# xindonglin99/allsteps_isaaclab

Measured on AMD Instinct MI355X. Metric: env-steps/sec (whole node), Allsteps-v0 at 4096 envs, 1/2/4/8 MI355X, higher is better.
Workload: dtype f32; 1 GPU; Allsteps-v0 biped walker, 4096 envs/GPU, stone curriculum level 0, decimation 4 x dt 1/240; num_envs_per_gpu=4096, global_envs=4096, parallelism=dp1 (env shards, no collective in step)

## Files before the change

### allsteps_isaaclab_amd/csrc/allsteps_abi.hip

```cpp
#include <hip/hip_runtime.h>

#include <algorithm>
#include <cstdlib>
#include <cstdio>
#include <cstring>
#include <string>
#include <vector>

#include "../../include/allsteps.h"
#include "allsteps_kernels.h"

namespace {

thread_local std::string g_err;

int fail(int code, const std::string& msg) {
  g_err = msg;
  return code;
}

#define HIP_TRY(expr)                                                                        \
  do {                                                                                       \
    hipError_t _e = (expr);                                                                  \
    if (_e != hipSuccess) return fail(AS_ERR_HIP, std::string(#expr ": ") + hipGetErrorString(_e)); \
// ... 123 lines not shown
  hipDeviceProp_t prop;
  HIP_TRY(hipGetDeviceProperties(&prop, device));
  if (std::strncmp(prop.gcnArchName, "gfx950", 6) != 0)
    return fail(AS_ERR_NO_DEVICE, std::string("as_create: device is ") + prop.gcnArchName + ", built for gfx950");

  as::Consts h{};
  h.model = *model;
  h.sim = *sim;
  h.task = *task;
  h.nv = 6 + model->num_hinges;
  h.act.mode = AS_ACT_TORQUE;
  h.st_has_hind = state->contact_mask_hind != nullptr;
  const int nl = model->num_links;
  for (int i = 0; i < nl; ++i) {
    int pa = model->parent[i];
    if (i == 0 ? pa != -1 : (pa < 0 || pa >= i)) return fail(AS_ERR_INVALID, "as_create: parent not topological");
    h.lpath[i] = (i == 0 ? 0u : h.lpath[pa]) | (1u << i);
    if (i > 0 && pa == 0) h.root_kids |= 1u << i;
  }
  for (int i = 0; i < nl; ++i)
    for (int l = 0; l < nl; ++l)
      if ((h.lpath[l] >> i) & 1u) h.lsub[i] |= 1u << l;
  for (int j = 0; j < h.nv; ++j) h.dsub[j] = j < 6 ? h.lsub[0] : h.lsub[j - 5];
  for (int i = 0; i < nl; ++i) {
    h.max_path = std::max(h.max_path, __builtin_popcount(h.lpath[i]) - 1);
    if (i > 0) h.max_sub = std::max(h.max_sub, __builtin_popcount(h.lsub[i]) - 1);
  }
  while ((1 << h.fk_rounds) < h.max_path) ++h.fk_rounds;
  if (h.fk_rounds > 4) return fail(AS_ERR_INVALID, "as_create: tree deeper than 16 links");
  for (int i = 0; i < nl; ++i) {
    int a = i > 0 ? model->parent[i] : 0;
    for (int r = 0; r < 4; ++r) {
      h.jump[i] |= (uint32_t)a << (8 * r);
      for (int k = 0; k < (1 << r); ++k) a = a > 0 ? model->parent[a] : 0;
    }
  }
  for (int k = 0; k < model->num_hinges; ++k) {
    int li = model->cfg_dof_link[k];
    if (li < 1 || li >= model->num_links) return fail(AS_ERR_INVALID, "as_create: cfg_dof_link");
  }
  for (int l = 0; l < model->num_links; ++l) {
    uint32_t mask = 0x3Fu;
    for (int i = l; i > 0; i = model->parent[i]) mask |= 1u << (6 + i - 1);
    h.ancmask[l] = mask;
  }
  for (int j = 0; j < h.nv; ++j)
    for (int k = 0; k < h.nv; ++k) {
      const int lk = k < 6 ? 0 : k - 5;
      if ((h.ancmask[lk] >> j) & 1u) h.ddesc[j] |= 1u << k;
    }
  if (!as::step_supported_nv(h.nv))
    return fail(AS_ERR_INVALID, "as_create: no k_step instantiation for " + std::to_string(h.nv) + " dofs");
  as::fill_lane_table(h);

  as_env* env = new as_env();
  env->n = num_envs;
  env->device = device;
  env->seed = seed;
  env->env_offset = env_id_offset;
  env->st = *state;
  env->num_steps = task->num_steps;
  env->nv = h.nv;
  env->host = h;
  env->sweep_skip = as_sweep_plan(model, nullptr) == 1;
  if (hipMalloc(&env->consts_dev, sizeof(as::Consts)) != hipSuccess ||
      hipMalloc(&env->counters_dev, 2 * as::kCntBank * sizeof(int32_t)) != hipSuccess ||
      hipMalloc(&env->side_dev, (size_t)as::kSideWords * num_envs * sizeof(uint32_t)) != hipSuccess) {
    (void)hipFree(env->consts_dev);
    (void)hipFree(env->counters_dev);
    delete env;
    return fail(AS_ERR_HIP, "as_create: hipMalloc failed");
  }
  HIP_TRY(hipMemcpy(env->consts_dev, &h, sizeof(as::Consts), hipMemcpyHostToDevice));
  HIP_TRY(hipMemset(env->counters_dev, 0, 2 * as::kCntBank * sizeof(int32_t)));
  HIP_TRY(hipMemset(env->side_dev, 0, (size_t)as::kSideWords * num_envs * sizeof(uint32_t)));
  const char* wm = std::getenv("ALLSTEPS_WAVE_MAP");
  if (as::wave_map_fits(num_envs) && !(wm && std::strcmp(wm, "0") == 0)) {
    env->map_streamed = num_envs / 2 > 8 * prop.multiProcessorCount && !(wm && std::strcmp(wm, "resident") == 0);
    std::vector<int32_t> map((size_t)num_envs);
    for (int w = 0; w < num_envs / as::kMapEnvs; ++w)
      for (int t = 0; t < as::kMapEnvs; ++t)
        map[(size_t)2 * as::wave_map_block(w, t >> 1, num_envs, env->map_streamed) + (t & 1)] = w * as::kMapEnvs + t;
    if (hipMalloc(&env->wave_map_dev, map.size() * sizeof(int32_t)) != hipSuccess) {
      (void)as_destroy(env);
      return fail(AS_ERR_HIP, "as_create: hipMalloc failed");
    }
    HIP_TRY(hipMemcpy(env->wave_map_dev, map.data(), map.size() * sizeof(int32_t), hipMemcpyHostToDevice));
  }
  *out = env;
  return AS_OK;
}

int as_destroy(as_env_t* env) {
  if (!env) return AS_OK;
  (void)hipSetDevice(env->device);
  for (hipEvent_t e : env->ev) (void)hipEventDestroy(e);
  (void)hipFree(env->consts_dev);
  (void)hipFree(env->counters_dev);
  (void)hipFree(env->side_dev);
  (void)hipFree(env->wave_map_dev);
  delete env;
  return AS_OK;
}

static int run(as_env_t* env, int mode, const float* actions, float* obs, float* reward, uint8_t* term,
               uint8_t* trunc, const float* reset_draws, void* stream, const uint8_t* reset_mask = nullptr) {
// ... 274 lines not shown
```

### allsteps_isaaclab_amd/csrc/allsteps_kernels.h

```cpp
#pragma once

#include <hip/hip_runtime.h>
#include <stdint.h>

#include "../../include/allsteps.h"
#include "allsteps_lane_table.h"

namespace as {

constexpr int kMaxLinks = 24;
constexpr int kMaxDofs = 6 + kMaxLinks - 1;

enum { kModeStep = 0, kModeReset = 1, kModePhysics = 2, kModeTask = 3 };

struct Consts {
  as_model_t model;
  as_sim_t sim;
  as_task_t task;
  as_actuator_t act;
  as_quad_task_t quad;
  int32_t nv;
  int32_t st_has_hind;
  int32_t max_path;
  int32_t max_sub;
  uint32_t root_kids;
  uint32_t lpath[kMaxLinks];
  uint32_t lsub[kMaxLinks];
  uint32_t ancmask[kMaxLinks];
  uint32_t dsub[kMaxDofs];
  uint32_t ddesc[kMaxDofs];
  uint32_t jump[kMaxLinks];
  int32_t fk_rounds;
  LaneRow lane[kLaneRows];
};
static_assert(kLaneRows == 32 && kMaxLinks <= kLaneRows && kMaxDofs <= kLaneRows, "one table row per k_step lane");
inline void fill_lane_table(Consts& c) {
  build_lane_table(c.lane, c.model, c.task, c.act, c.nv, c.lpath, c.lsub, c.ancmask, c.dsub, c.jump);
}

struct StepArgs {
  const Consts* consts;
  as_state_t st;
  int32_t n;
  int32_t mode;
  const float* actions;
  float* reward;
  float* obs;
  uint32_t* side;
  uint8_t* terminated;
  uint8_t* truncated;
  const float* reset_draws;
  const uint8_t* reset_mask;
  int32_t* counters;
  uint64_t seed;
  int64_t env_offset;
  unsigned long long* stamps;
  const int32_t* wave_map;
};

enum {
  kStLoad = 0, kStFK, kStLinkQ, kStDyn, kStChol, kStSolve, kStCollide, kStRows, kStWsolve, kStPGS,
  kStIntegrate, kStFKFinal, kStTask, kStReset, kStStore, kNumStamps
};

constexpr int kCntSlots = 16;
constexpr int kCntStride = 16;
constexpr int kCntBank = kCntStride * (1 + kCntSlots);

constexpr int kSideState = 9;
constexpr int kSideObs = 11;
constexpr int kSideRegen = kSideState + kSideObs;
constexpr int kSideCost = kSideRegen + 1;
constexpr int kSideWords = kSideCost + 1;

constexpr int kMapEnvs = 64;
__host__ __device__ inline bool wave_map_fits(int n) { return n > 0 && n % (8 * kMapEnvs) == 0; }
__host__ __device__ inline int wave_map_block(int w, int p, int n, bool streamed) {
  const int C = n / kMapEnvs;
  if (streamed || p < kMapEnvs / 4) return p * C + w;
  return (n >> 2) + (kMapEnvs / 2 - 1 - p) * C + w;
}
constexpr int kCntLevel = 2;
constexpr int kCntDropped = 3;

struct QuadArgs {
// ... 63 lines not shown
```

### allsteps_isaaclab_amd/csrc/allsteps_kernels.hip

```cpp
#include <hip/hip_runtime.h>

#include "../../include/allsteps.h"
#include "allsteps_device.h"
#include "allsteps_kernels.h"

namespace as {

constexpr int G = 32;
constexpr int EPB = 2;
constexpr int LMAX = kMaxLinks;
constexpr int NVMAX = 6 + LMAX - 1;
constexpr int MAXC = AS_MAX_CONTACTS;
constexpr int MAXR = AS_MAX_ROWS;
constexpr int NST = AS_NUM_STONES;
constexpr int kBisectIters = 12;
constexpr int kPairsPerChunk = G;
static_assert(kPairsPerChunk - 1 + G <= 64, "pending pair list (PhaseScratch::col.pl)");
constexpr int kSweepB = 4;
typedef float v4f __attribute__((ext_vector_type(4)));
typedef float v2f __attribute__((ext_vector_type(2)));

static_assert(NVMAX <= G, "one lane per generalized velocity");
static_assert(LMAX <= G, "one lane per link");
static_assert(MAXR <= G, "one row per lane in the row builders");
// ... 155 lines not shown

__device__ __forceinline__ int half_scan3(int c, int& total) {
  const int sh = threadIdx.x & 32;
  const uint32_t m0 = (uint32_t)(__ballot((c & 1) != 0) >> sh);
  const uint32_t m1 = (uint32_t)(__ballot((c & 2) != 0) >> sh);
  const uint32_t lt = (1u << (threadIdx.x & 31)) - 1u;
  total = __popc(m0) + 2 * __popc(m1);
  return __popc(m0 & lt) + 2 * __popc(m1 & lt);
}

template <int CTRL>
__device__ __forceinline__ uint32_t dpp_u(uint32_t v) {
  return (uint32_t)__builtin_amdgcn_update_dpp(0, (int)v, CTRL, 0xF, 0xF, true);
}

__device__ __forceinline__ void half_or2(uint32_t& x, uint32_t& y) {
  const auto s = __builtin_amdgcn_permlane16_swap((int)x, (int)y, false, false);
  uint32_t c = (uint32_t)s[0] | (uint32_t)s[1];
  c |= dpp_u<0xB1>(c);
  c |= dpp_u<0x4E>(c);
  c |= dpp_u<0x141>(c);
  c |= dpp_u<0x140>(c);
  const auto t = __builtin_amdgcn_permlane16_swap((int)c, (int)c, false, false);
  x = (uint32_t)t[0];
  y = (uint32_t)t[1];
}

template <int N>
__device__ __forceinline__ void half_min_n(float (&v)[N]) {
  static_assert(N % 2 == 0, "pairs");
  constexpr int P = N / 2;
  float c[P];
#pragma unroll
  for (int p = 0; p < P; ++p) {
    const auto s = __builtin_amdgcn_permlane16_swap(__float_as_int(v[2 * p]), __float_as_int(v[2 * p + 1]), false, false);
    c[p] = fminf(__int_as_float(s[0]), __int_as_float(s[1]));
  }
#pragma unroll
  for (int p = 0; p < P; ++p) c[p] = fminf(c[p], dpp<0xB1>(c[p]));
#pragma unroll
  for (int p = 0; p < P; ++p) c[p] = fminf(c[p], dpp<0x4E>(c[p]));
#pragma unroll
  for (int p = 0; p < P; ++p) c[p] = fminf(c[p], dpp<0x141>(c[p]));
#pragma unroll
  for (int p = 0; p < P; ++p) c[p] = fminf(c[p], dpp<0x140>(c[p]));
#pragma unroll
  for (int p = 0; p < P; ++p) {
    const auto s = __builtin_amdgcn_permlane16_swap(__float_as_int(c[p]), __float_as_int(c[p]), false, false);
    v[2 * p] = __int_as_float(s[0]);
    v[2 * p + 1] = __int_as_float(s[1]);
  }
}

constexpr int kWaveRecFlag = 31, kWaveRecBase = 64, kWaveRecWords = 26;
static_assert(16 + kNumStamps <= kWaveRecFlag && kNumStamps + 11 <= kWaveRecWords, "stamp slots");
struct Stamp {
  unsigned long long* p;
  unsigned long long* acc;
  unsigned long long t;
  unsigned long long t0 = 0ull, rt0 = 0ull;
  unsigned rows = 0u, cons = 0u;
  __device__ void start() {
    if (p) {
      if (threadIdx.x < kNumStamps) acc[threadIdx.x] = 0ull;
      t = t0 = __builtin_amdgcn_s_memtime();
      rt0 = __builtin_amdgcn_s_memrealtime();
      __syncthreads();
    }
  }
  __device__ void count(int nrow, int nc) {
    if (p) {
      rows += (unsigned)nrow;
      cons += (unsigned)nc;
    }
  }
  __device__ void mark(int k) {
    if (p) {
      unsigned long long now = __builtin_amdgcn_s_memtime();
      if (threadIdx.x == 0) acc[k] += now - t;
      t = now;
    }
  }
  __device__ void flush() {
    if (p) {
      __syncthreads();
      unsigned long long tot = 0;
      for (int k = 0; k < kNumStamps; ++k) tot += acc[k];
      if (p[kWaveRecFlag]) {
        unsigned long long* rec = p + kWaveRecBase + (size_t)blockIdx.x * kWaveRecWords;
        const unsigned long long now = __builtin_amdgcn_s_memtime();
        const unsigned hw = __builtin_amdgcn_s_getreg((31 << 11) | 4);
        const unsigned xcc = __builtin_amdgcn_s_getreg((31 << 11) | 20);
        const int k = threadIdx.x;
        if (k < kNumStamps) rec[k] = acc[k];
        if (k == 0) {
          rec[kNumStamps] = tot; rec[kNumStamps + 1] = t0; rec[kNumStamps + 2] = now;
          rec[kNumStamps + 9] = rt0; rec[kNumStamps + 10] = __builtin_amdgcn_s_memrealtime();
          rec[kNumStamps + 3] = hw; rec[kNumStamps + 4] = xcc;
          rec[kNumStamps + 5] = rows; rec[kNumStamps + 7] = cons;
        }
        if (k == 32) { rec[kNumStamps + 6] = rows; rec[kNumStamps + 8] = cons; }
      } else {
        if (threadIdx.x < kNumStamps) {
          atomicAdd(p + threadIdx.x, acc[threadIdx.x]);
          atomicMax(p + 16 + threadIdx.x, acc[threadIdx.x]);
        }
        if (threadIdx.x == 0) atomicMax(p + kNumStamps, tot);
      }
    }
  }
};

__device__ __forceinline__ int take_bit(uint32_t& m, bool& valid) {
  valid = m != 0u;
  const int l = valid ? __builtin_ctz(m) : 0;
  m &= m - 1u;
  return l;
}

constexpr int kZeroRow = LMAX - 1;
static_assert(AS_ACT_DIM + 1 <= kZeroRow, "zero row past the links");
__device__ __forceinline__ int take_bit_z(uint32_t& m) {
  const int l = m != 0u ? __builtin_ctz(m) : kZeroRow;
  m &= m - 1u;
  return l;
}

template <int W, int U>
__device__ __forceinline__ void path_sum(uint32_t mask, int n_max, float (&acc)[W], const float (*rows)[W]) {
  for (int it = 0; it < n_max; it += U) {
    int l[U];
#pragma unroll
    for (int u = 0; u < U; ++u) l[u] = take_bit_z(mask);
    float x[U][W];
#pragma unroll
    for (int u = 0; u < U; ++u)
#pragma unroll
      for (int k = 0; k < W; ++k) x[u][k] = rows[l[u]][k];
#pragma unroll
    for (int u = 0; u < U; ++u)
#pragma unroll
      for (int k = 0; k < W; ++k) acc[k] += x[u][k];
  }
}

struct LinkC {
  float oq[4], ax[3], an[3], op[3];
};
__device__ __forceinline__ LinkC load_link(const Consts& K, int lane) {
  const as_model_t& m = K.model;
  const int i = lane >= 1 && lane < m.num_links ? lane : 0;
  LinkC c;
#pragma unroll
  for (int k = 0; k < 4; ++k) c.oq[k] = m.offset_quat[i][k];
// ... 455 lines not shown
                             const float* n, float sep, float r) {
  if (slot >= ncap) return;
  s.clink[slot] = link; s.clink2[slot] = link2; s.cstone[slot] = stone; s.cfoot[slot] = foot; s.csep[slot] = sep;
  for (int k = 0; k < 3; ++k) { s.cn[slot][k] = n[k]; s.cpt[slot][k] = P[k] - n[k] * r; }
}

struct GeomC {
  int link, type, foot;
  float r, p0[3], p1[3];
  uint32_t anc;
};
__device__ __forceinline__ float capsule_contact_sel(const float* a1, const float* b1, float r1, const float* a2,
                                                     const float* b2, float r2, float* P, float* n) {
  float d1[3], d2[3], r[3];
#pragma unroll
  for (int k = 0; k < 3; ++k) {
    d1[k] = b1[k] - a1[k];
    d2[k] = b2[k] - a2[k];
    r[k] = a1[k] - a2[k];
  }
  const float a = as_dot3(d1, d1), e = as_dot3(d2, d2), f = as_dot3(d2, r);
  const float eps = 1e-12f;
  const bool pa = a <= eps, pe = e <= eps, gen = !pa && !pe;
  const float c = as_dot3(d1, r);
  const float b = as_dot3(d1, d2);
  const float den = fmaf(a, e, -(b * b));
  const float sm = den > 0.f ? as_clamp01(fmaf(b, f, -(c * e)) / den) : 0.f;
  const float tq = (pa ? f : fmaf(b, sm, f)) / e;
  const bool lo = gen && tq < 0.f, hi = gen && tq > 1.f;
  const float sq = as_clamp01((hi ? b - c : -c) / a);
  const float s = pa ? 0.f : (pe || lo || hi) ? sq : sm;
  const float t = pa ? (pe ? 0.f : as_clamp01(tq)) : pe ? 0.f : lo ? 0.f : hi ? 1.f : tq;
  float c1[3], c2[3], w[3];
#pragma unroll
  for (int k = 0; k < 3; ++k) {
    c1[k] = fmaf(s, d1[k], a1[k]);
    c2[k] = fmaf(t, d2[k], a2[k]);
    w[k] = c1[k] - c2[k];
  }
  const float dist = sqrtf(as_dot3(w, w));
  const bool nz = dist > 1e-9f;
  const float inv = 1.0f / dist;
  n[0] = nz ? w[0] * inv : 0.f;
  n[1] = nz ? w[1] * inv : 0.f;
  n[2] = nz ? w[2] * inv : 1.f;
  const float sep = dist - r1 - r2;
  const float off = fmaf(0.5f, sep, r2);
#pragma unroll
  for (int k = 0; k < 3; ++k) P[k] = fmaf(off, n[k], c2[k]);
  return sep;
}

__device__ __forceinline__ int collide(const Consts& K, EnvS& s, int lane, int ncap, const GeomC& gc, const float* h,
                                       float margin) {
  const as_model_t& m = K.model;
  const int nst = K.task.num_steps, ng = m.num_geoms, npri = m.num_priority_geoms, nsp = m.num_self_pairs;
  constexpr int kSelfW = AS_MAX_SELF_PAIRS / G;
  int spw[kSelfW];
#pragma unroll
  for (int i = 0; i < kSelfW; ++i) spw[i] = G * i + lane < nsp ? m.self_pair[G * i + lane] : 0;
  const bool gv = lane < ng;
  const int link = gc.link, gtype = gc.type, foot = gc.foot;
  const float r = gc.r;
  float a[3], bb[3];
  {
    float t0[3], t1[3];
    matvec3(s.R[link], gc.p0, t0);
    matvec3(s.R[link], gc.p1, t1);
    for (int k = 0; k < 3; ++k) { a[k] = s.p[link][k] + t0[k]; bb[k] = s.p[link][k] + t1[k]; }
  }
  const float L = sqrtf((bb[0] - a[0]) * (bb[0] - a[0]) + (bb[1] - a[1]) * (bb[1] - a[1]) +
                        (bb[2] - a[2]) * (bb[2] - a[2]));
  const float mid[3] = {0.5f * (a[0] + bb[0]), 0.5f * (a[1] + bb[1]), 0.5f * (a[2] + bb[2])};
  float blo[3], bhi[3], ext[6];
#pragma unroll
  for (int k = 0; k < 3; ++k) {
    const float e = gtype == 0 ? a[k] : fminf(a[k], bb[k]);
    const float f = gtype == 0 ? a[k] : fmaxf(a[k], bb[k]);
    ext[k] = gv ? e - r : 1e30f;
    ext[3 + k] = gv ? -(f + r) : 1e30f;
  }
  half_min_n(ext);
#pragma unroll
  for (int k = 0; k < 3; ++k) {
    blo[k] = ext[k] - margin;
    bhi[k] = -ext[3 + k] + margin;
  }
  bool isc = false;
  float cst[3] = {0.f, 0.f, 0.f};
  if (lane < nst) {
    isc = true;
#pragma unroll
    for (int k = 0; k < 3; ++k) {
      cst[k] = s.stones[3 * lane + k] - s.root_pos[k];
      isc = isc && (cst[k] - h[k] <= bhi[k]) && (cst[k] + h[k] >= blo[k]);
    }
  }
  uint64_t bal = __ballot(isc);
  const int half = (threadIdx.x >> 5) & 1;
  uint32_t mine = (uint32_t)(bal >> (32 * half));
  if (isc) {
    const int pos = __popc(mine & ((1u << lane) - 1u));
    s.cand[pos] = lane;
    *reinterpret_cast<v4f*>(s.x.col.cc[pos]) = v4f{cst[0], cst[1], cst[2], 0.f};
  }
  const int ncand = __popc(mine);
  {
// ... 26 lines not shown
    for (int k = 0; k < 3; ++k) c[k] = s.stones[3 * pst + k] - s.root_pos[k];
    float lo = 0.f, hi = 1.f;
#pragma unroll 4
    for (int it = 0; it < kBisectIters; ++it) {
      const float t = 0.5f * (lo + hi);
      const bool up = sd_box_slope(A, Bb, t, c, h) > 0.f;
      hi = up ? t : hi;
      lo = up ? lo : t;
    }
    if (act) {
      float n0[3];
      const float s0 = sd_box(A, c, h, n0) - pr;
      if (pty == 0) {
        if (s0 < margin) {
          for (int k = 0; k < 3; ++k) { P0[k] = A[k]; N0[k] = n0[k]; }
          SEP0 = s0;
          cnt = 1;
        }
      } else {
        float n1[3];
        float s1 = sd_box(Bb, c, h, n1) - pr;
        float ts = 0.5f * (lo + hi), Ps[3], ns[3];
        for (int k = 0; k < 3; ++k) Ps[k] = A[k] + ts * (Bb[k] - A[k]);
        float ss = sd_box(Ps, c, h, ns) - pr;
        bool e0 = s0 < margin, e1 = s1 < margin;
        bool es = ss < margin && ss < fminf(s0, s1) - 0.002f;
        for (int k = 0; k < 3; ++k) { P0[k] = A[k]; N0[k] = n0[k]; }
        SEP0 = s0;
        if (e0) {
          for (int k = 0; k < 3; ++k) { P1[k] = Bb[k]; N1[k] = n1[k]; P2[k] = Ps[k]; N2[k] = ns[k]; }
          SEP1 = s1; SEP2 = ss;
          if (!e1) { for (int k = 0; k < 3; ++k) { P1[k] = Ps[k]; N1[k] = ns[k]; } SEP1 = ss; }
        } else {
          for (int k = 0; k < 3; ++k) { P0[k] = Bb[k]; N0[k] = n1[k]; P1[k] = Ps[k]; N1[k] = ns[k]; }
          SEP0 = s1; SEP1 = ss;
          if (!e1) { for (int k = 0; k < 3; ++k) { P0[k] = Ps[k]; N0[k] = ns[k]; } SEP0 = ss; }
        }
        cnt = (int)e0 + (int)e1 + (int)es;
      }
    }
    int total;
    const int slot = base + half_scan3(cnt, total);
    if (cnt > 0) emit_contact(s, slot, ncap, plink, -1, pst, pfoot, P0, N0, SEP0, pr);
    if (cnt > 1) emit_contact(s, slot + 1, ncap, plink, -1, pst, pfoot, P1, N1, SEP1, pr);
    if (cnt > 2) emit_contact(s, slot + 2, ncap, plink, -1, pst, pfoot, P2, N2, SEP2, pr);
    base += total;
    const int rest = pend - npairs;
    const int tail = lane < rest ? pl[npairs + lane] : 0;
    __syncthreads();
    if (lane < rest) pl[lane] = tail;
    pend = rest;
    __syncthreads();
  };
  __syncthreads();
  uint32_t* cneed = s.x.col.need;
  const float pa[3] = {gtype == 0 ? a[0] : mid[0], gtype == 0 ? a[1] : mid[1], gtype == 0 ? a[2] : mid[2]};
  const float cap_lim = 0.5f * L + r + margin;
#pragma unroll 1
  for (int ci = 0; ci < ncand; ++ci) {
    const v4f cv = *reinterpret_cast<const v4f*>(s.x.col.cc[ci]);
    const float c[3] = {cv.x, cv.y, cv.z};
    float nr[3];
    const float sd = sd_box(pa, c, h, nr);
    bool need = false;
    if (gv) need = gtype == 0 ? sd - r < margin : sd <= cap_lim;
    const uint32_t bl = (uint32_t)(__ballot(need) >> (32 * half));
    if (lane == 0) cneed[ci] = bl;
  }
  __syncthreads();
  const uint32_t primask = npri >= 32 ? ~0u : (1u << npri) - 1u;
  const int wcand = max(__builtin_amdgcn_readlane(ncand, 0), __builtin_amdgcn_readlane(ncand, 32));
#pragma unroll 1
  for (int cls = 0; cls < 2; ++cls) {
#pragma unroll 1
    for (int ci = 0; ci < wcand; ++ci) {
      const uint32_t bl = ci < ncand ? cneed[ci] & (cls == 0 ? primask : ~primask) : 0u;
      if ((bl >> lane) & 1u) pl[pend + __popc(bl & ((1u << lane) - 1u))] = (s.cand[ci] << 8) | lane;
      pend += __popc(bl);
      if (max(__builtin_amdgcn_readlane(pend, 0), __builtin_amdgcn_readlane(pend, 32)) >= kPairsPerChunk)
        flush(pend < kPairsPerChunk ? pend : kPairsPerChunk);
    }
  }
  if (pend > 0) flush(pend);
  pend = 0;
  auto flush_self = [&](int npairs) {
    const bool act = lane < npairs;
    const int e = pl[act ? lane : 0];
    const int g1 = e & 0xff, g2 = e >> 8;
    int cnt = 0, l1 = 0, l2 = 0;
    float P[3], n[3], sep = 0.f;
    if (act) {
      const float* q1 = s.x.col.g[g1];
      const float* q2 = s.x.col.g[g2];
      sep = capsule_contact_sel(q1, q1 + 3, q1[6], q2, q2 + 3, q2[6], P, n);
      cnt = sep < margin;
      l1 = __float_as_int(q1[7]) >> 8;
      l2 = __float_as_int(q2[7]) >> 8;
    }
    int total;
    const int slot = base + half_scan3(cnt, total);
    if (cnt) emit_contact(s, slot, ncap, l1, l2, -1, -1, P, n, sep, 0.f);
    base += total;
    const int rest = pend - npairs;
    const int tail = lane < rest ? pl[npairs + lane] : 0;
    __syncthreads();
    if (lane < rest) pl[lane] = tail;
    pend = rest;
    __syncthreads();
  };
  uint32_t hbl[kSelfW];
  static_assert(kSelfW % 4 == 0, "batches of four words");
#pragma unroll
  for (int i = 0; i < kSelfW; ++i) hbl[i] = 0u;
#pragma unroll
  for (int i0 = 0; i0 < kSelfW; i0 += 4) {
    if (G * i0 >= nsp) break;
    v4f s1[4], s2[4];
#pragma unroll
    for (int i = 0; i < 4; ++i) {
      s1[i] = *reinterpret_cast<const v4f*>(s.x.col.bs[spw[i0 + i] & 0xff]);
      s2[i] = *reinterpret_cast<const v4f*>(s.x.col.bs[spw[i0 + i] >> 8]);
    }
    asm volatile("" : "+v"(s1[0]), "+v"(s1[1]), "+v"(s1[2]), "+v"(s1[3]), "+v"(s2[0]), "+v"(s2[1]), "+v"(s2[2]),
                 "+v"(s2[3]));
#pragma unroll
    for (int i = 0; i < 4; ++i) {
      const bool pv = G * (i0 + i) + lane < nsp;
      const float m1[3] = {s1[i].x, s1[i].y, s1[i].z}, m2[3] = {s2[i].x, s2[i].y, s2[i].z};
      const bool hit = as_sphere_bound(m1, s1[i].w, m2, s2[i].w, margin);
      hbl[i0 + i] = (uint32_t)(__ballot(pv & hit) >> (32 * half));
    }
  }
  const uint32_t lt = (1u << lane) - 1u;
  int tot = 0, at[kSelfW];
#pragma unroll
  for (int i = 0; i < kSelfW; ++i) {
// ... 192 lines not shown
    s.tau[lane] = as_dc_motor(s.qt[lane], s.qi[lane], s.u[6 + lane], A.stiffness, A.damping, A.saturation_effort,
                              A.effort_limit, A.velocity_limit);
  }
  fk<true>(K, s, lane, tp, lc, smp);
  ts.mark(kStFK);
  float Sj[6], Fj[6];
  dynamics<NV>(K, s, lane, tp, K.sim.gravity, Sj, Fj, smp);
  ts.mark(kStLinkQ);
  typedef SweepLayout<NV> SL;
  constexpr int NP = SL::NP;
  float Hr[NP];
  h_row<NV>(s, lane, tp, gc.anc, Sj, Fj, *reinterpret_cast<float(*)[NV]>(Hr));
  ts.mark(kStDyn);
  {
    float Hs[NP];
#pragma unroll
    for (int k = 0; k < NV; ++k) Hs[SL::pos(SL::padded(k))] = Hr[k];
#pragma unroll
    for (int q = 0; q < NP - NV; ++q) Hs[SL::pos(SL::PAD + q)] = lane == NV + q ? 1.f : 0.f;
    sweep_inverse<NV, SKIP>(s, lane, Hs);
#pragma unroll
    for (int k = 0; k < NV; ++k) Hr[k] = lane < NV ? -Hs[SL::pos(SL::padded(k))] : 0.f;
#pragma unroll
    for (int k = NV; k < NP; ++k) Hr[k] = 0.f;
  }
  ts.mark(kStChol);
  float uj = 0.f;
  {
    float acc = 0.f;
#pragma unroll
    for (int k = 0; k < NV; ++k) acc = fmaf(Hr[k], s.b[k], acc);
    if (lane < NV) {
      uj = fmaf(dt, acc, s.u[lane]);
      s.u[lane] = uj;
    }
  }
  __syncthreads();
  ts.mark(kStSolve);
  int lo_v = 0, hi_v = 0;
  float err_lo = 0.f, err_hi = 0.f;
  if (lane < nh) {
    float qv = s.qi[lane], pred = qv + dt * s.u[6 + lane];
    err_lo = tp.lo - qv;
    err_hi = qv - tp.hi;
    lo_v = pred < tp.lo;
    hi_v = pred > tp.hi;
  }
  int ltotal;
  const int lpos = half_scan3(lo_v + hi_v, ltotal);
  const int nlim = ltotal < MAXR ? ltotal : MAXR;
  const int ncap = (MAXR - nlim) / 3 < MAXC ? (MAXR - nlim) / 3 : MAXC;
  float sb = K.sim.baumgarte, ssl = K.sim.slop, smd = K.sim.max_depen_vel, sfr = K.sim.friction, smg = K.sim.margin;
  float sh[3] = {K.sim.stone_half[0], K.sim.stone_half[1], K.sim.stone_half[2]};
  asm volatile("" : "+s"(sb), "+s"(ssl), "+s"(smd), "+s"(sfr), "+s"(smg), "+s"(sh[0]), "+s"(sh[1]), "+s"(sh[2]));
  const int nc = collide(K, s, lane, ncap, gc, sh, smg);
  ts.mark(kStCollide);

  if (lane < nc) {
    float t1[3], t2[3];
    tangents(s.cn[lane], t1, t2);
    const float* dirs[3] = {s.cn[lane], t1, t2};
    float sp = s.csep[lane];
    const int lk = s.clink[lane] | ((s.clink2[lane] + 1) << 8);
    for (int d = 0; d < 3; ++d) {
      int r = 3 * lane + d;
      for (int k = 0; k < 3; ++k) s.cdir[lane][d][k] = dirs[d][k];
      s.rlink[r] = lk;
      s.rsign[r] = 0.f;
      const float num = sp < 0.f ? sb * fmaxf(-sp - ssl, 0.f) : -sp;
      const float tv = num / dt;
      s.rmeta[r][1] = d == 0 ? (sp < 0.f ? fminf(tv, smd) : tv) : 0.f;
      s.rmeta[r][2] = d == 1 ? sfr : 0.f;
    }
  }
  const int crow = 3 * nc;
  int slot = crow + lpos;
  for (int sd = 0; sd < 2; ++sd) {
    int viol = sd == 0 ? lo_v : hi_v;
    if (!viol) continue;
    if (slot < MAXR) {
      float err = sd == 0 ? err_lo : err_hi;
      s.rlink[slot] = -1 - (6 + lane);
      s.rsign[slot] = sd == 0 ? 1.f : -1.f;
      const float tv = (err > 0.f ? sb * err : err) / dt;
      s.rmeta[slot][1] = err > 0.f ? fminf(tv, smd) : tv;
      s.rmeta[slot][2] = slot % 3 == 2 ? __builtin_inff() : 0.f;
    }
    ++slot;
  }
  const int nrow = crow + nlim;
  ts.count(nrow, nc);
  if (lane == 0) s.nrows += nrow;
  const int maxrow = max(__builtin_amdgcn_readlane(nrow, 0), __builtin_amdgcn_readlane(nrow, 32));
  __syncthreads();
  {
    const int lvl = __builtin_amdgcn_readfirstlane(maxrow) / kPrioRows;
    if (lvl >= 3) __builtin_amdgcn_s_setprio(3);
    else if (lvl == 2) __builtin_amdgcn_s_setprio(2);
    else if (lvl == 1) __builtin_amdgcn_s_setprio(1);
    else __builtin_amdgcn_s_setprio(0);
  }
  v2f Jr[LDJ / 2];
  uint32_t jmask = ~0u;
  {
    const int rr = lane < MAXR ? lane : 0;
    const int c = rr / 3, u = rr - 3 * c;
    const int lk = s.rlink[rr];
    const float sg = s.rsign[rr];
// ... 95 lines not shown
    half_or2(b[2], b[3]);
#pragma unroll
    for (int k = 0; k < 4; ++k) mask_out[k] = b[k];
  }
  float rq[4], rp[3];
  {
    const float* u = s.u;
    float c0w[3];
    for (int k = 0; k < 3; ++k) c0w[k] = fmaf(dt, u[k], s.root_pos[k] + s.c0[k]);
    const float* w = u + 3;
    const float wn = sqrtf(dot3(w, w));
    const float th = wn * dt;
    float sn, cs;
    as_sincosf(0.5f * th, &sn, &cs);
    const float sc = sn / wn;
    const bool big = th > 1e-12f;
    const float dq[4] = {big ? cs : 1.f, big ? w[0] * sc : 0.5f * dt * w[0], big ? w[1] * sc : 0.5f * dt * w[1],
                         big ? w[2] * sc : 0.5f * dt * w[2]};
    const float* q0 = s.root_quat;
    float nq[4] = {dq[0] * q0[0] - dq[1] * q0[1] - dq[2] * q0[2] - dq[3] * q0[3],
                   dq[0] * q0[1] + dq[1] * q0[0] + dq[2] * q0[3] - dq[3] * q0[2],
                   dq[0] * q0[2] - dq[1] * q0[3] + dq[2] * q0[0] + dq[3] * q0[1],
                   dq[0] * q0[3] + dq[1] * q0[2] - dq[2] * q0[1] + dq[3] * q0[0]};
    const float qn = 1.0f / sqrtf(nq[0] * nq[0] + nq[1] * nq[1] + nq[2] * nq[2] + nq[3] * nq[3]);
    for (int k = 0; k < 4; ++k) rq[k] = nq[k] * qn;
    float Rn[9], cl[3];
    quat_to_mat(rq, Rn);
    matvec3(Rn, m.com[0], cl);
    for (int k = 0; k < 3; ++k) rp[k] = c0w[k] - cl[k];
  }
  if (lane < nh) {
    float v = fminf(fmaxf(s.u[6 + lane], -K.sim.max_joint_vel), K.sim.max_joint_vel);
    s.u[6 + lane] = v;
    s.qi[lane] = fmaf(dt, v, s.qi[lane]);
  }
  if (lane == 0) {
    for (int k = 0; k < 4; ++k) s.root_quat[k] = rq[k];
    for (int k = 0; k < 3; ++k) s.root_pos[k] = rp[k];
  }
  __syncthreads();
  ts.mark(kStIntegrate);
}


struct Useful {
  float h, roll, pitch, body_dist, dist_s;
  int reached;
};

template <class TaskT>
__device__ void compute_useful(TaskT& T, const float* root_pos, const float* root_quat, const float* bp,
                               const float* stones_env, int stride, uint32_t mask_r, uint32_t mask_l, int& idx,
                               int& prev, int& next, int& count, int& swing, float& pot, float& old_pot,
                               float* foot_contact, bool tick, Useful& u) {
  const int N = T.num_steps;
  float lower = fminf(bp[8], bp[5]);
  u.h = bp[2] - lower;
  euler_rp_from_quat(root_quat, &u.roll, &u.pitch);
  u.reached = 0;
  u.dist_s = 0.f;
  if (tick) {
    float cf0 = ((mask_r >> idx) & 1u) ? 1.f : 0.f;
    float cf1 = ((mask_l >> idx) & 1u) ? 1.f : 0.f;
    foot_contact[0] = cf0;
    foot_contact[1] = cf1;
    float tx = stones_env[(idx * 3 + 0) * stride], ty = stones_env[(idx * 3 + 1) * stride];
    float dx0 = bp[3] - tx, dy0 = bp[4] - ty, dx1 = bp[6] - tx, dy1 = bp[7] - ty;
    float d0 = sqrtf(dx0 * dx0 + dy0 * dy0), d1 = sqrtf(dx1 * dx1 + dy1 * dy1);
    float cfs = swing == 0 ? cf0 : cf1;
    float ds = swing == 0 ? d0 : d1;
    u.reached = (cfs > 0.f) && (ds < T.step_radius);
    if (u.reached) count += 1;
    if (count >= T.stop_frames) {
      swing ^= 1;
      int ni = min(max(idx + 1, 0), N - 1);
      idx = ni;
      prev = min(max(ni - 1, 0), N - 1);
      next = min(max(ni + 1, 0), N - 1);
      count = 0;
    }
    u.dist_s = swing == 0 ? d0 : d1;
  }
  float dx = stones_env[(next * 3 + 0) * stride] - root_pos[0];
  float dy = stones_env[(next * 3 + 1) * stride] - root_pos[1];
  u.body_dist = sqrtf(dx * dx + dy * dy);
  old_pot = pot;
  pot = -(u.body_dist) / T.step_dt;
}

__device__ __forceinline__ int xcd_block(int b, int nb) {
  const int q = nb >> 3, r = nb & 7, x = b & 7, slot = b >> 3;
  return (x < r ? x * (q + 1) : r * (q + 1) + (x - r) * q) + slot;
}

constexpr int kStepThreads = 64;
static_assert(kStepThreads == 64, "k_step assumes a one-wave (wave64) workgroup: see the FK rounds");

template <int NV, uint64_t SKIP>
__global__ __launch_bounds__(kStepThreads) __attribute__((amdgpu_waves_per_eu(2, 2))) void k_step(StepArgs P) {
  __shared__ Smem sm;
  CK* Kc = (CK*)P.consts;
  const Consts& K = *(const Consts*)Kc;
  const int el = threadIdx.x >> 5, lane = threadIdx.x & 31;
  const int n = P.n;
  EnvS& s = sm.env[el];
  const as_state_t& st = P.st;
  Stamp ts{P.stamps, sm.stamp_acc, 0ull};
  ts.start();
  int e_raw = xcd_block(blockIdx.x, gridDim.x) * EPB + el;
  if (P.wave_map) e_raw = P.wave_map[EPB * blockIdx.x + el];
  const ConstV4* rowp = (const ConstV4*)&Kc->lane[lane];
// ... 66 lines not shown
  if (lane < 4) s.root_quat[lane] = v_rq;
  if (lane == 0) { s.ndrop = 0; s.nrows = 0; }
  if (lane < nh) {
    int i = (int)rc[9].w - 1;
    s.qi[i] = v_q;
    s.u[6 + i] = v_qd;
    float a = fminf(fmaxf(v_a, -1.f), 1.f);
    s.act[lane] = a;
    s.tau[i] = gain * row_gear * a;
    s.qt[i] = Kc->act.action_scale * a + row_dq;
  }
  if (lane < ns3) s.stones[lane] = v_s0;
  if (lane + G < ns3) s.stones[lane + G] = v_s1;
  if (lane < kPkWords) s.pk[lane] = v_pk;
  __syncthreads();
  ts.mark(kStLoad);
  const bool do_physics = P.mode == kModeStep || P.mode == kModePhysics;
  if (do_physics) {
    const int substeps = Kc->sim.substeps;
    for (int sub = 0; sub < substeps; ++sub) substep<NV, SKIP>(K, sm, s, lane, tp, gc, lc, mask, ts);
  }
  const u32x4* rowg = (const u32x4*)&K.lane[lane];
  const u32x4 rr8 = rowg[8], rr9 = rowg[9];
  const float rs_q = __uint_as_float(rr8.z), rs_qm = __uint_as_float(rr8.w), rs_sg = __uint_as_float(rr9.x);
  const float rs_lo = __uint_as_float(rr9.y), rs_hi = __uint_as_float(rr9.z);
  const int rs_li = (int)rr9.w;
  float rd_m = 0.f, rd_n = 0.f;
  if (P.reset_draws && P.mode != kModePhysics) {
    rd_m = P.reset_draws[(size_t)e * 22];
    rd_n = P.reset_draws[(size_t)e * 22 + 1 + lh];
  }
  asm volatile("" ::: "memory");
  if (do_physics) {
    fk<false>(*Kc, s, lane, tp, lc, Kc->max_path);
    if (lane == 0) { s.mask[0] = mask[0]; s.mask[1] = mask[1]; s.mask[2] = mask[2]; s.mask[3] = mask[3]; }
  }
  ts.mark(kStFKFinal);
  if (lane == 0 && !do_physics) { s.mask[0] = mask[0]; s.mask[1] = mask[1]; }
  __syncthreads();
  float bp[9];
  if (do_physics) {
    const int ls[3] = {m.torso_link, m.foot_link[0], m.foot_link[1]};
    for (int b = 0; b < 3; ++b)
      for (int k = 0; k < 3; ++k) bp[3 * b + k] = s.root_pos[k] + s.p[ls[b]][k];
  } else {
    for (int k = 0; k < 9; ++k) bp[k] = __uint_as_float(s.pk[kPkBody + k]);
  }
  int idx = (int)s.pk[kPkIdx], prev = (int)s.pk[kPkPrev], next = (int)s.pk[kPkNext], count = (int)s.pk[kPkCount];
  int swing = (int)s.pk[kPkSwing], ep_len = (int)s.pk[kPkEpLen];
  float pot = __uint_as_float(s.pk[kPkPot]), old_pot = __uint_as_float(s.pk[kPkOldPot]);
  float fc[2] = {__uint_as_float(s.pk[kPkFc0]), __uint_as_float(s.pk[kPkFc1])};
  uint32_t episode = s.pk[kPkEpisode];
  bool done = false;
  if (P.mode == kModeStep || P.mode == kModeTask) {
    ep_len += 1;
    Useful u;
    compute_useful(T, s.root_pos, s.root_quat, bp, s.stones, 1, s.mask[0], s.mask[1], idx, prev, next, count,
                   swing, pot, old_pot, fc, true, u);
    float a2 = 0.f, en = 0.f;
    int atlim = 0;
    if (lane < nh) {
      const int li = rs_li;
      float a = s.act[lane];
      a2 = a * a;
      en = fabsf(s.u[6 + li - 1] * a);
      atlim = fabsf(scale_transform(s.qi[li - 1], rs_lo, rs_hi)) > 0.99f;
    }
    a2 = half_sum(a2);
    en = half_sum(en);
    uint64_t bl = __ballot(atlim != 0);
    int nlim = __popcll(bl >> (32 * el) & 0xffffffffull);
    const float* lv = s.u;
    float speed = sqrtf(lv[0] * lv[0] + lv[1] * lv[1] + lv[2] * lv[2]);
    bool time_out = ep_len >= T.max_episode_length - 1;
    bool fell = u.h < term_h;
    bool so_fast = speed > 5.0f;
    bool died = s.root_pos[2] < T.fall_abs;
    bool terminated = fell || so_fast || died;
    float progress = pot - old_pot;
    bool roll_v = (u.roll > 0.4f) || (u.roll < -0.4f);
    bool pitch_v = (u.pitch > 0.4f) || (u.pitch < -0.2f);
    float roll_cost = roll_v ? fabsf(u.roll) : 0.f;
    float pitch_cost = pitch_v ? fabsf(u.pitch) : 0.f;
    float speed_cost = speed > 1.6f ? speed - 1.6f : 0.f;
    float action_cost = T.action * sqrtf(a2);
    float energy_cost = T.energy * en;
    float limit_cost = (float)nlim * T.joint_limit;
    bool cond = u.reached && count == 1 && idx < T.num_steps - 1;
    float step_rew = cond ? 50.0f * as_expf(-u.dist_s / 0.25f) : 0.f;
    bool bonus_c = idx == T.num_steps - 1 && u.body_dist < 0.15f;
    float total = T.alive + progress;
    total = total - roll_cost;
    total = total - pitch_cost;
    total = total - speed_cost;
    total = total - energy_cost;
    total = total - action_cost;
    total = total - limit_cost;
    total = total + step_rew;
    total = total + (bonus_c ? 10.0f : 0.f);
    float rew = terminated ? T.death : total;
    done = terminated || time_out;
    if (valid && lane == 0) {
      P.reward[e] = rew;
      P.terminated[e] = terminated ? 1 : 0;
      P.truncated[e] = time_out ? 1 : 0;
    }
  } else if (P.mode == kModeReset) {
    done = P.reset_mask == nullptr || P.reset_mask[e] != 0;
  }
// ... 19 lines not shown
      float dm = rd_m, dn = rd_n;
      if (!P.reset_draws) {
        float blk[4];
        philox_block(P.seed, (uint32_t)(P.env_offset + e), episode, 0u, kResetTag, blk);
        dm = blk[0];
        if (lane < nh) {
          const int k = 1 + lane;
          philox_block(P.seed, (uint32_t)(P.env_offset + e), episode, (uint32_t)(k >> 2), kResetTag, blk);
          const int sl = k & 3;
          dn = sl == 0 ? blk[0] : (sl == 1 ? blk[1] : (sl == 2 ? blk[2] : blk[3]));
        }
      }
      ep_len = 0;
      old_pot = 0.f; pot = 0.f; count = 0; swing = 0; idx = 1; prev = 0; next = 2;
      const bool mirror = dm > 0.5f;
      if (mirror) swing ^= 1;
      if (lane < nh) {
        const float sign = mirror ? rs_sg : 1.f;
        float jp = mirror ? rs_qm : rs_q;
        float jv = 0.f * sign;
        int li = rs_li;
        float x = jp + (dn * (T.noise_hi - T.noise_lo) + T.noise_lo);
        float sc = fminf(fmaxf(scale_transform(x, rs_lo, rs_hi), T.clip_lo), T.clip_hi);
        s.qi[li - 1] = unscale_transform(sc, rs_lo, rs_hi);
        s.u[6 + li - 1] = jv;
      }
      if (lane < 3) {
        const float ir[3] = {T.init_root[0], T.init_root[1], T.init_root[2]};
        s.root_pos[lane] = lane == 0 ? ir[0] : (lane == 1 ? ir[1] : ir[2]);
        s.u[lane] = 0.f;
        s.u[3 + lane] = 0.f;
      }
      if (lane == 0) {
        float sg = mirror ? -1.f : 1.f;
        s.root_quat[0] = 1.f;
        s.root_quat[1] = 0.f * sg;
        s.root_quat[2] = 0.f * sg;
        s.root_quat[3] = 0.f * sg;
      }
      episode += 1u;
    }
    __syncthreads();
    fk<false>(*Kc, s, lane, tp, lc, Kc->max_path);
    if (done) {
      const int ls[3] = {m.torso_link, m.foot_link[0], m.foot_link[1]};
      for (int b = 0; b < 3; ++b)
        for (int k = 0; k < 3; ++k) bp[3 * b + k] = s.root_pos[k] + s.p[ls[b]][k];
    }
  }
  __syncthreads();
  if (P.obs) {
    int i2 = idx, p2 = prev, n2 = next, c2 = count, w2 = swing;
    float pot2 = pot, op2 = old_pot, fc2[2] = {fc[0], fc[1]};
    Useful u2;
    compute_useful(T, s.root_pos, s.root_quat, bp, s.stones, 1, s.mask[0], s.mask[1], i2, p2, n2, c2, w2, pot2,
                   op2, fc2, true, u2);
    float* ob = s.x.obs;
    uint32_t* side = P.side;
    if (lane == 0) {
      ob[0] = u2.h;
      ob[1] = u2.roll;
      ob[2] = u2.pitch;
      float vb[3];
      quat_rotate_inverse(s.root_quat, s.u, vb);
      ob[3] = vb[0]; ob[4] = vb[1]; ob[5] = vb[2];
      ob[48] = fc2[0];
      ob[49] = fc2[1];
    }
    if (lane < nh) {
      const int li = rs_li;
      ob[6 + lane] = scale_transform(s.qi[li - 1], rs_lo, rs_hi);
      ob[27 + lane] = fminf(fmaxf(s.u[6 + li - 1] * T.dof_vel_scale, -5.f), 5.f);
    }
    if (lane < 6) {
      const int t = lane < 3 ? lane : lane - 3;
      const int ti = lane < 3 ? (t == 0 ? p2 : (t == 1 ? i2 : n2)) : (t == 0 ? prev : (t == 1 ? idx : next));
      const float tw[3] = {s.stones[3 * ti], s.stones[3 * ti + 1], s.stones[3 * ti + 2]};
      float o3[3];
      subtract_frame_transforms(s.root_pos, s.root_quat, tw, o3);
      if (lane < 3) {
        for (int k = 0; k < 3; ++k) ob[50 + 3 * t + k] = o3[k];
      } else if (valid) {
        for (int k = 0; k < 3; ++k) side[(kSideState + 2 + 3 * t + k) * n + e] = __float_as_uint(o3[k]);
      }
    }
    __syncthreads();
    if (valid) {
      float* orow = P.obs + (size_t)e * AS_OBS_DIM;
      orow[lane] = ob[lane];
      if (lane < AS_OBS_DIM - 32) orow[32 + lane] = ob[32 + lane];
      if (lane == 0) {
        const uint32_t sv[kSideState + 2] = {(uint32_t)idx, (uint32_t)prev, (uint32_t)next, (uint32_t)count,
                                             (uint32_t)swing, __float_as_uint(pot), __float_as_uint(old_pot),
                                             __float_as_uint(fc[0]), __float_as_uint(fc[1]),
                                             __float_as_uint(fc[0]), __float_as_uint(fc[1])};
        for (int k = 0; k < kSideState + 2; ++k) side[k * n + e] = sv[k];
        side[kSideRegen * n + e] = regen ? 1u : 0u;
      }
    }
    idx = i2; prev = p2; next = n2; count = c2; swing = w2;
    pot = pot2; old_pot = op2; fc[0] = fc2[0]; fc[1] = fc2[1];
  }
  ts.mark(kStReset);
  if (valid) {
    if (lane < 3) {
      st.root_pos[lane * n + e] = s.root_pos[lane];
      st.root_lin[lane * n + e] = s.u[lane];
      st.root_ang[lane * n + e] = s.u[3 + lane];
    }
// ... 584 lines not shown
```

Before: 34.79 million env-steps/s.

## Split bisection of leftover collision pairs across lane groups

```diff
diff --git a/allsteps_isaaclab_amd/csrc/allsteps_abi.hip b/allsteps_isaaclab_amd/csrc/allsteps_abi.hip
--- a/allsteps_isaaclab_amd/csrc/allsteps_abi.hip
+++ b/allsteps_isaaclab_amd/csrc/allsteps_abi.hip
@@ -199,6 +199,12 @@
   if (!as::step_supported_nv(h.nv))
     return fail(AS_ERR_INVALID, "as_create: no k_step instantiation for " + std::to_string(h.nv) + " dofs");
   as::fill_lane_table(h);
+  h.pair_group_cap = 4;
+  if (const char* pg = std::getenv("ALLSTEPS_PAIR_GROUP")) {
+    if (std::strlen(pg) != 1 || pg[0] < '1' || pg[0] > '4')
+      return fail(AS_ERR_INVALID, std::string("as_create: ALLSTEPS_PAIR_GROUP=") + pg + ", expected 1, 2, 3 or 4");
+    h.pair_group_cap = pg[0] - '0';
+  }
 
   as_env* env = new as_env();
   env->n = num_envs;
diff --git a/allsteps_isaaclab_amd/csrc/allsteps_kernels.h b/allsteps_isaaclab_amd/csrc/allsteps_kernels.h
--- a/allsteps_isaaclab_amd/csrc/allsteps_kernels.h
+++ b/allsteps_isaaclab_amd/csrc/allsteps_kernels.h
@@ -5,6 +5,7 @@
 
 #include "../../include/allsteps.h"
 #include "allsteps_lane_table.h"
+#include "allsteps_pair_group.h"
 
 namespace as {
 
@@ -31,6 +32,7 @@
   uint32_t ddesc[kMaxDofs];
   uint32_t jump[kMaxLinks];
   int32_t fk_rounds;
+  int32_t pair_group_cap;
   LaneRow lane[kLaneRows];
 };
 static_assert(kLaneRows == 32 && kMaxLinks <= kLaneRows && kMaxDofs <= kLaneRows, "one table row per k_step lane");
diff --git a/allsteps_isaaclab_amd/csrc/allsteps_kernels.hip b/allsteps_isaaclab_amd/csrc/allsteps_kernels.hip
--- a/allsteps_isaaclab_amd/csrc/allsteps_kernels.hip
+++ b/allsteps_isaaclab_amd/csrc/allsteps_kernels.hip
@@ -231,14 +231,14 @@
   }
 }
 
-constexpr int kWaveRecFlag = 31, kWaveRecBase = 64, kWaveRecWords = 26;
-static_assert(16 + kNumStamps <= kWaveRecFlag && kNumStamps + 11 <= kWaveRecWords, "stamp slots");
+constexpr int kWaveRecFlag = 31, kWaveRecBase = 64, kWaveRecWords = 30;
+static_assert(16 + kNumStamps <= kWaveRecFlag && kNumStamps + 14 <= kWaveRecWords, "stamp slots");
 struct Stamp {
   unsigned long long* p;
   unsigned long long* acc;
   unsigned long long t;
   unsigned long long t0 = 0ull, rt0 = 0ull;
-  unsigned rows = 0u, cons = 0u;
+  unsigned rows = 0u, cons = 0u, prs = 0u, lvls = 0u;
   __device__ void start() {
     if (p) {
       if (threadIdx.x < kNumStamps) acc[threadIdx.x] = 0ull;
@@ -251,6 +251,13 @@
     if (p) {
       rows += (unsigned)nrow;
       cons += (unsigned)nc;
+    }
+  }
+  __device__ void pairs(int np, int level) {
+    if (p) {
+      const unsigned mx = prs >> 16 > (unsigned)np ? prs >> 16 : (unsigned)np;
+      prs = ((prs + (unsigned)np) & 0xffffu) | (mx << 16);
+      lvls += 1u << (8 * (level < 2 ? 0 : level - 1));
     }
   }
   __device__ void mark(int k) {
@@ -277,8 +284,9 @@
           rec[kNumStamps + 9] = rt0; rec[kNumStamps + 10] = __builtin_amdgcn_s_memrealtime();
           rec[kNumStamps + 3] = hw; rec[kNumStamps + 4] = xcc;
           rec[kNumStamps + 5] = rows; rec[kNumStamps + 7] = cons;
+          rec[kNumStamps + 11] = prs; rec[kNumStamps + 13] = lvls;
         }
-        if (k == 32) { rec[kNumStamps + 6] = rows; rec[kNumStamps + 8] = cons; }
+        if (k == 32) { rec[kNumStamps + 6] = rows; rec[kNumStamps + 8] = cons; rec[kNumStamps + 12] = prs; }
       } else {
         if (threadIdx.x < kNumStamps) {
           atomicAdd(p + threadIdx.x, acc[threadIdx.x]);
@@ -840,7 +848,7 @@
 }
 
 __device__ __forceinline__ int collide(const Consts& K, EnvS& s, int lane, int ncap, const GeomC& gc, const float* h,
-                                       float margin) {
+                                       float margin, int gcap, Stamp& ts) {
   const as_model_t& m = K.model;
   const int nst = K.task.num_steps, ng = m.num_geoms, npri = m.num_priority_geoms, nsp = m.num_self_pairs;
   constexpr int kSelfW = AS_MAX_SELF_PAIRS / G;
@@ -973,6 +981,55 @@
     pend = rest;
     __syncthreads();
   };
+  auto flush_grp = [&](int npairs, int L) {
+    const int gm = (1 << L) - 1, k = lane & gm, pi = lane >> L;
+    const bool act = pi < npairs;
+    const int e = act ? pl[pi] : 0;
+    const int gi = e & 0xff, pst = e >> 8;
+    const float* gq = s.x.col.g[gi];
+    const float A[3] = {gq[0], gq[1], gq[2]}, Bb[3] = {gq[3], gq[4], gq[5]};
+    const float pr = gq[6];
+    const int meta = __float_as_int(gq[7]);
+    const int pty = meta & 15, pfoot = ((meta >> 4) & 15) - 1, plink = meta >> 8;
+    float c[3];
+    for (int i = 0; i < 3; ++i) c[i] = s.stones[3 * pst + i] - s.root_pos[i];
+    float lo = 0.f, d = 1.f;
+    const float sc = pair_group_scale(L);
+    const int g0 = (threadIdx.x & 63) & ~gm;
+#pragma unroll 1
+    for (int it = 0; it < kBisectIters; it += L) {
+      const float w = d * sc;
+      const bool up = sd_box_slope(A, Bb, pair_group_point(lo, w, k), c, h) > 0.f;
+      pair_group_walk(lo, w, L, (uint32_t)(__ballot(up) >> g0));
+      d = w;
+    }
+    const float tm = 0.5f * (lo + (lo + d));
+    float Q[3], nq[3];
+    const uint32_t m0 = k == 0 ? ~0u : 0u, m1 = k == 1 ? ~0u : 0u;
+    for (int i = 0; i < 3; ++i) {
+      const uint32_t ps = __float_as_uint(A[i] + tm * (Bb[i] - A[i]));
+      const uint32_t b1 = (__float_as_uint(Bb[i]) & m1) | (ps & ~m1);
+      Q[i] = __uint_as_float((__float_as_uint(A[i]) & m0) | (b1 & ~m0));
+    }
+    const float sv = sd_box(Q, c, h, nq) - pr;
+    const float smin = fminf(dpp<0x112>(sv), dpp<0x111>(sv));
+    const bool cap = pty != 0;
+    const bool sel = (k == 0) | (cap & (k == 1)) | (cap & (k == 2) & (sv < smin - 0.002f));
+    const int cnt = (int)(act & (sv < margin) & sel);
+    int total;
+    const int slot = base + half_scan3(cnt, total);
+    if (cnt) emit_contact(s, slot, ncap, plink, -1, pst, pfoot, Q, nq, sv, pr);
+    base += total;
+    pend -= npairs;
+    __syncthreads();
+  };
+  static_assert(kBisectIters == kPairGroupIters, "allsteps_pair_group.h: the group rounds cover kBisectIters");
+  auto flush_any = [&](int wpend) {
+    const int L = pair_group_level(wpend, gcap);
+    const int np = pend < kPairsPerChunk ? pend : kPairsPerChunk;
+    ts.pairs(np, L);
+    if (L) flush_grp(np, L); else flush(np);
+  };
   __syncthreads();
   uint32_t* cneed = s.x.col.need;
   const float pa[3] = {gtype == 0 ? a[0] : mid[0], gtype == 0 ? a[1] : mid[1], gtype == 0 ? a[2] : mid[2]};
@@ -992,17 +1049,18 @@
   const uint32_t primask = npri >= 32 ? ~0u : (1u << npri) - 1u;
   const int wcand = max(__builtin_amdgcn_readlane(ncand, 0), __builtin_amdgcn_readlane(ncand, 32));
 #pragma unroll 1
-  for (int cls = 0; cls < 2; ++cls) {
+  for (int cls = 0; cls < 3; ++cls) {
+    const int nci = cls < 2 ? wcand : 1;
 #pragma unroll 1
-    for (int ci = 0; ci < wcand; ++ci) {
-      const uint32_t bl = ci < ncand ? cneed[ci] & (cls == 0 ? primask : ~primask) : 0u;
+    for (int ci = 0; ci < nci; ++ci) {
+      const uint32_t bl = cls < 2 && ci < ncand ? cneed[ci] & (cls == 0 ? primask : ~primask) : 0u;
       if ((bl >> lane) & 1u) pl[pend + __popc(bl & ((1u << lane) - 1u))] = (s.cand[ci] << 8) | lane;
       pend += __popc(bl);
-      if (max(__builtin_amdgcn_readlane(pend, 0), __builtin_amdgcn_readlane(pend, 32)) >= kPairsPerChunk)
-        flush(pend < kPairsPerChunk ? pend : kPairsPerChunk);
-    }
-  }
-  if (pend > 0) flush(pend);
+      const int wpend = max(__builtin_amdgcn_readlane(pend, 0), __builtin_amdgcn_readlane(pend, 32));
+      const bool appending = cls < 2;
+      if (appending ? wpend >= kPairsPerChunk : wpend > 0) flush_any(wpend);
+    }
+  }
   pend = 0;
   auto flush_self = [&](int npairs) {
     const bool act = lane < npairs;
@@ -1301,8 +1359,10 @@
   const int ncap = (MAXR - nlim) / 3 < MAXC ? (MAXR - nlim) / 3 : MAXC;
   float sb = K.sim.baumgarte, ssl = K.sim.slop, smd = K.sim.max_depen_vel, sfr = K.sim.friction, smg = K.sim.margin;
   float sh[3] = {K.sim.stone_half[0], K.sim.stone_half[1], K.sim.stone_half[2]};
-  asm volatile("" : "+s"(sb), "+s"(ssl), "+s"(smd), "+s"(sfr), "+s"(smg), "+s"(sh[0]), "+s"(sh[1]), "+s"(sh[2]));
-  const int nc = collide(K, s, lane, ncap, gc, sh, smg);
+  int gcap = K.pair_group_cap;
+  asm volatile("" : "+s"(sb), "+s"(ssl), "+s"(smd), "+s"(sfr), "+s"(smg), "+s"(sh[0]), "+s"(sh[1]), "+s"(sh[2]),
+               "+s"(gcap));
+  const int nc = collide(K, s, lane, ncap, gc, sh, smg, gcap, ts);
   ts.mark(kStCollide);
 
   if (lane < nc) {
@@ -1504,11 +1564,13 @@
 __device__ void compute_useful(TaskT& T, const float* root_pos, const float* root_quat, const float* bp,
                                const float* stones_env, int stride, uint32_t mask_r, uint32_t mask_l, int& idx,
                                int& prev, int& next, int& count, int& swing, float& pot, float& old_pot,
-                               float* foot_contact, bool tick, Useful& u) {
+                               float* foot_contact, bool tick, Useful& u, bool pose = true) {
   const int N = T.num_steps;
-  float lower = fminf(bp[8], bp[5]);
-  u.h = bp[2] - lower;
-  euler_rp_from_quat(root_quat, &u.roll, &u.pitch);
+  if (pose) {
+    float lower = fminf(bp[8], bp[5]);
+    u.h = bp[2] - lower;
+    euler_rp_from_quat(root_quat, &u.roll, &u.pitch);
+  }
   u.reached = 0;
   u.dist_s = 0.f;
   if (tick) {
@@ -1681,9 +1743,9 @@
   float fc[2] = {__uint_as_float(s.pk[kPkFc0]), __uint_as_float(s.pk[kPkFc1])};
   uint32_t episode = s.pk[kPkEpisode];
   bool done = false;
+  Useful u{};
   if (P.mode == kModeStep || P.mode == kModeTask) {
     ep_len += 1;
-    Useful u;
     compute_useful(T, s.root_pos, s.root_quat, bp, s.stones, 1, s.mask[0], s.mask[1], idx, prev, next, count,
                    swing, pot, old_pot, fc, true, u);
     float a2 = 0.f, en = 0.f;
@@ -1809,9 +1871,9 @@
   if (P.obs) {
     int i2 = idx, p2 = prev, n2 = next, c2 = count, w2 = swing;
     float pot2 = pot, op2 = old_pot, fc2[2] = {fc[0], fc[1]};
-    Useful u2;
+    Useful u2 = u;
     compute_useful(T, s.root_pos, s.root_quat, bp, s.stones, 1, s.mask[0], s.mask[1], i2, p2, n2, c2, w2, pot2,
-                   op2, fc2, true, u2);
+                   op2, fc2, true, u2, any_done || !(P.mode == kModeStep || P.mode == kModeTask));
     float* ob = s.x.obs;
     uint32_t* side = P.side;
     if (lane == 0) {
diff --git a/allsteps_isaaclab_amd/csrc/allsteps_pair_group.h b/allsteps_isaaclab_amd/csrc/allsteps_pair_group.h
--- /dev/null
+++ b/allsteps_isaaclab_amd/csrc/allsteps_pair_group.h
@@ -0,0 +1,40 @@
+#pragma once
+
+#include <math.h>
+#include <stdint.h>
+
+#if defined(__HIPCC__) || defined(__CUDACC__)
+#define AS_PG_FN __host__ __device__ __forceinline__
+#else
+#define AS_PG_FN inline
+#endif
+
+namespace as {
+
+constexpr int kPairGroupIters = 12;
+
+AS_PG_FN float pair_group_scale(int L) { return L == 4 ? 0.0625f : (L == 3 ? 0.125f : 0.25f); }
+
+AS_PG_FN int pair_group_level(int npairs, int cap) {
+  const int L = npairs <= 2 ? 4 : (npairs <= 4 ? 3 : (npairs <= 8 ? 2 : 0));
+  const int Lc = L < cap ? L : cap;
+  return Lc >= 2 ? Lc : 0;
+}
+
+AS_PG_FN float pair_group_point(float lo, float w, int k) { return fmaf((float)(k + 1), w, lo); }
+
+AS_PG_FN int pair_group_step(int li, uint32_t b2, int half) {
+  const int mi = li + half;
+  return ((b2 >> mi) & 1u) != 0u ? li : mi;
+}
+AS_PG_FN void pair_group_walk(float& lo, float w, int L, uint32_t bits) {
+  const uint32_t b2 = bits << 1;
+  const int n = 1 << L;
+  int li = pair_group_step(0, b2, n >> 1);
+  li = pair_group_step(li, b2, n >> 2);
+  li = pair_group_step(li, b2, n >> 3);
+  li = pair_group_step(li, b2, n >> 4);
+  lo = fmaf((float)li, w, lo);
+}
+
+}
```

After: 35.50 million env-steps/s (median of 6 runs). +2.0%, better.
